# zovoilis-lab/Flye

Measured on AMD Instinct MI355X. Metric: Gbp reads overlapped/sec, higher is better.
Workload: dtype u64

## Files before the change

### flye_amd/csrc/fg_api.hip

```cpp
#include "fg_ctx.h"
#include <chrono>
#include <cmath>

#include <algorithm>
#include <new>

#include <mutex>
#include <atomic>

static std::mutex g_poolMutex;
static std::vector<BatchOwner*> g_pool;

BatchOwner* BatchOwner::acquire()
{
	std::lock_guard<std::mutex> lock(g_poolMutex);
	if (g_pool.empty()) return new BatchOwner;
	BatchOwner* b = g_pool.back();
	g_pool.pop_back();
	return b;
}

void BatchOwner::release(BatchOwner* b)
{
	if (!b) return;
// ... 562 lines not shown
		n > (1ULL << 40))
		return FG_ERR_ARG;
	return guarded(c, [&]()
	{
		HIP_CHECK(hipSetDevice(c->device));
		fgDebugScan(c, data, n, elem_bytes, inclusive != 0, in_place != 0);
	});
}

int fg_debug_radix_sort_pairs(fg_ctx* c, uint64_t* keys, uint64_t* vals, uint64_t n, int begin_bit, int end_bit,
							  int* passes_run)
{
	if (!c || (n && (!keys || !vals)) || begin_bit < 0 || end_bit > 64 || begin_bit > end_bit || n > (1ULL << 30) - 1 ||
		((uintptr_t)keys & 7u) || ((uintptr_t)vals & 7u))
		return FG_ERR_ARG;
	if (passes_run) *passes_run = 0;
	return guarded(c, [&]()
	{
		HIP_CHECK(hipSetDevice(c->device));
		fgDebugRadixSortPairs(c, keys, vals, n, begin_bit, end_bit, passes_run);
	});
}

int fg_debug_probe_skip_check(fg_ctx* c, uint64_t* clear_bits, uint64_t* violations)
{
	if (!c || !clear_bits || !violations) return FG_ERR_ARG;
	return guarded(c, [&]()
	{
		HIP_CHECK(hipSetDevice(c->device));
		if (!c->indexBuilt) throw FgError{FG_ERR_STATE, "no index"};
		u64 cb = 0, vi = 0;
		fgDebugProbeSkipCheck(c, &cb, &vi);
		*clear_bits = cb; *violations = vi;
	});
}

int fg_debug_edit_distances(fg_ctx* c, uint32_t n_pairs, int use_hpc, int32_t* out_dist, int32_t* out_len_a,
							int32_t* out_len_b)
{
	if (!c || (n_pairs && (!out_dist || !out_len_a || !out_len_b))) return FG_ERR_ARG;
	return guarded(c, [&]()
	{
		HIP_CHECK(hipSetDevice(c->device));
		fgDebugEditDistances(c, n_pairs, use_hpc, out_dist, out_len_a, out_len_b);
	});
}

namespace {
struct CigarOwner {
	std::vector<uint64_t> runOff;
	std::vector<uint8_t> ops;
	std::vector<int32_t> lens;
	std::vector<float> err;
};
}

int fg_align_cigar_ksw(fg_ctx* c, uint32_t n_pairs, const uint8_t* trg, const uint64_t* trg_off, const uint8_t* qry,
					   const uint64_t* qry_off, struct fg_cigar_batch* out)
{
	if (!c || !out || !trg_off || !qry_off || (trg_off[n_pairs] && !trg) || (qry_off[n_pairs] && !qry)) return FG_ERR_ARG;
	memset(out, 0, sizeof(*out));
	CigarOwner* own = nullptr;
	const int rc = guarded(c, [&]()
	{
		HIP_CHECK(hipSetDevice(c->device));
		std::vector<u64> runOff;
// ... 692 lines not shown
```

### flye_amd/csrc/fg_chain.hip

```cpp
#include "fg_wavesort.h"

#include <algorithm>

#define WG 256
#define I32_MIN ((i32)0x80000000)

struct ChainParams {
	int k, maxJump, minOverlap, maxOverhang;
	int checkOverhang, forceLocal;
	float minUnique;
	u32 firstId;
	u32 qFirstId;
	int onlyMaxExt;
	int keepAln;
	int ablate;
};

namespace {

struct CandAcc {
	typedef int4 T;
	int4* c;
	__device__ int4 load(int i) const { return c[i]; }
	__device__ void store(int i, const int4& x) { c[i] = x; }
	__device__ bool less(const int4& a, const int4& b) const { return a.w > b.w; }
};

__device__ __forceinline__ bool overlap_test(const ChainParams& P, u32 curId, u32 extId, i32 curLen,
											 i32 extLen, i32 cb, i32 ce, i32 eb, i32 ee)
{
	const i32 curRange = ce - cb, extRange = ee - eb;
	if (curRange < P.minOverlap || extRange < P.minOverlap) return false;
	const float lengthDiff = (float)abs(curRange - extRange);
	if (lengthDiff > 0.5f * (float)min(curRange, extRange)) return false;
	if (curId == extId)
	{
		const i32 inter = min(ce, ee) - max(cb, eb);
		if (inter > curRange / 2) return false;
	}
	if (curId == (extId ^ 1u))
	{
		const i32 inter = min(ce, extLen - eb) - max(cb, extLen - ee);
		if (inter > curRange / 2) return false;
	}
	if (!P.forceLocal && P.checkOverhang)
	{
		const i32 ovh = max(min(cb, eb), min(curLen - ce, extLen - ee));
		if (ovh > P.maxOverhang) return false;
// ... 431 lines not shown
			}
			else
			{
#pragma unroll
				for (int r = 0; r < R; ++r)
				{
					const u32 o = (u32)__shfl_xor((int)v[r], j);
					const bool asc = (((r * 64 + lane) & k) == 0);
					const bool lower = (lane & j) == 0;
					v[r] = (asc == lower) ? min(v[r], o) : max(v[r], o);
				}
			}
		}
	}
	bool tie = false;
	i32 nLive = 0;
#pragma unroll
	for (int r = 0; r < R; ++r)
	{
		u32 nx = (u32)__shfl_down((int)v[r], 1);
		const u32 first = r + 1 < R ? (u32)__builtin_amdgcn_readlane((int)v[r + 1 < R ? r + 1 : r], 0) : 0xFFFFFFFFu;
		if (lane == 63) nx = first;
		tie |= nx != 0xFFFFFFFFu && (nx >> 10) == (v[r] >> 10);
		nLive += __popcll(__builtin_amdgcn_ballot_w64(v[r] != 0xFFFFFFFFu));
	}
	if (__builtin_amdgcn_ballot_w64(tie)) return -1;
#pragma unroll
	for (int r = 0; r < R; ++r)
		if (v[r] != 0xFFFFFFFFu) oval[r * 64 + lane] = v[r] & 1023u;
	return nLive;
}


template <bool USE_LDS, int BT_CAP>
__device__ __forceinline__ void finish_group(const ChainParams& P, const i32 n, const u32 curId, const u32 extId, const i32 curLen,
											 const i32 extLen, const u32* cur, const u32* ext, i32* score, i32* back, u32* okey, u32* oval,
											 unsigned short* plLds, int* stack, int* small, i32* btLds, int4* cd, u32* primCountG)
{
	const int lane = threadIdx.x & 63;
	const int k = P.k;
	i32 nOrder = -1;
	if (USE_LDS && !(P.ablate & 64))
	{
		if (n <= 64) nOrder = fast_score_order<1>(n, score, back, oval);
		else if (n <= 128) nOrder = fast_score_order<2>(n, score, back, oval);
		else if (n <= 256) nOrder = fast_score_order<4>(n, score, back, oval);
	}
	const bool exact = nOrder < 0;
	if (exact)
	{
		for (i32 i = lane; i < n; i += 64) { okey[i] = (u32)(0x7fffffff - score[i]); oval[i] = (u32)i; }
		nOrder = n;
	}
	wsort::wave_mem_fence();
	if (exact && !(P.ablate & 2))
	{
		if (USE_LDS)
			wsort::wave_sort<u32, unsigned short>(okey, oval, n, plLds, plLds + n, stack, small);
		else if (BT_CAP > 0 && n <= BT_CAP)
		{
			unsigned short* pl = (unsigned short*)btLds;
			wsort::wave_sort<u32, unsigned short>(okey, oval, n, pl, pl + BT_CAP, stack, small);
		}
		else wsort::wave_sort<u32, u32>(okey, oval, n, oval + n, oval + 2 * n, stack, small);
	}

	if (P.ablate & 8) return;
	if (!USE_LDS && P.keepAln)
	{
		i32* bc = (i32*)(oval + n);
		for (i32 i = lane; i < n; i += 64) bc[i] = back[i];
		back = bc;
	}
// ... 269 lines not shown

u32 fetchU32(fg_ctx* c, const u32* dptr)
{
	u32 v;
	HIP_CHECK(hipMemcpyAsync(&v, dptr, 4, hipMemcpyDeviceToHost, c->stream));
	HIP_CHECK(hipStreamSynchronize(c->stream));
	return v;
}

}

u32 fgChainSmallMax()
{
	if (getenv("FG_CHAIN_FUSED") && atoi(getenv("FG_CHAIN_FUSED")) == 0) return 0u;
	return getenv("FG_FUSED_CAP") ? (u32)std::max(64, std::min(1024, atoi(getenv("FG_FUSED_CAP")))) : (u32)FIN_CAP_S;
}

void fgChainStage(fg_ctx* c, const fg_detector_params* p, uint8_t forceLocal, u64 nGroups, u64 nHits, int keyMode,
				  int curBits)
{
	hipStream_t s = c->stream;
	ChainParams cp;
	cp.k = c->k; cp.maxJump = p->max_jump; cp.minOverlap = p->min_overlap; cp.maxOverhang = p->max_overhang;
	cp.checkOverhang = p->max_overhang > 0; cp.forceLocal = forceLocal ? 1 : 0;
	{
		const float minKmerSruvivalRate = 0.01;
		cp.minUnique = minKmerSruvivalRate * p->min_overlap;
	}
	cp.firstId = c->firstId;
	cp.qFirstId = c->hasQ ? c->qFirstId : c->firstId;
	cp.onlyMaxExt = p->only_max_ext ? 1 : 0;
	cp.keepAln = p->keep_alignment ? 1 : 0;
	cp.ablate = getenv("FG_ABLATE") ? atoi(getenv("FG_ABLATE")) : 0;
	if (!nGroups) return;
	const i32* qLen = c->hasQ ? c->dQLen.p : c->dLen.p;
	u32 minSize = 0;
	while ((float)minSize < cp.minUnique) ++minSize;
	if (minSize == 0) minSize = 1;
	c->dListSmall.reserve(nGroups + 1); c->dListBig.reserve(nGroups + 1); c->dListDp.reserve(nGroups + 1);
	c->dGroupExtSorted.reserve(nGroups + 1);
	c->dListCnt.reserve(4);
	const u64 hitCap = std::max<u64>(nHits, c->hitCapHint);
	c->dCur.reserve(hitCap + 16); c->dExt.reserve(hitCap + 16);
	c->dScore.reserve(hitCap + 16); c->dBack.reserve(hitCap + 16);
	c->dTmp32.reserve(4 * hitCap + 16);
	c->dCand.reserve(hitCap + 1);
	const unsigned gridG = (unsigned)((nGroups + (u64)WG * LIST_ITEMS - 1) / ((u64)WG * LIST_ITEMS));
	const u32 fusedMax = fgChainSmallMax();
	const bool fused = fusedMax != 0;
	if (fused) c->dListFused.reserve(nGroups + 1);
	HIP_CHECK(hipMemsetAsync(c->dListCnt.p, 0, 16, s));
	{ ScopedK t(c->timer, "k_group_list");
	  hipLaunchKernelGGL(k_group_list, gridG, WG, 0, s, nGroups, nHits, c->dGroupStart.p, minSize, c->dGroupFirstCur.p,
						 c->dGroupLastCur.p, (i32)p->min_overlap, c->dListSmall.p, c->dListBig.p, (u32)PREP_CAP,
						 c->dListFused.p, fusedMax, c->dListCnt.p, c->dPrimFlag.p, c->dDpSize.p); }
	u32 nPrep[4];
	c->hScalar.reserve(8);
	HIP_CHECK(hipMemcpyAsync(c->hScalar.p, c->dListCnt.p, 16, hipMemcpyDeviceToHost, s));
	HIP_CHECK(hipStreamSynchronize(s));
	memcpy(nPrep, c->hScalar.p, 16);
	const u32 nFused = fused ? nPrep[2] : 0u;
	if (!nPrep[0] && !nPrep[1] && !nFused) return;
	if (fused)
	{
		const bool others = nPrep[0] || nPrep[1];
		const bool sideStreams = !(getenv("FG_CHAIN_STREAMS") && atoi(getenv("FG_CHAIN_STREAMS")) == 1);
// ... 199 lines not shown
```

### flye_amd/csrc/fg_ctx.h

```cpp
#pragma once

#include <hip/hip_runtime.h>
#include <cstdint>
#include <cstdio>
#include <cstdlib>
#include <new>
#include <cstring>
#include <string>
#include <vector>
#include <map>
#include <memory>
#include <condition_variable>
#include <functional>
#include <mutex>
#include <thread>
#include <atomic>
#include <algorithm>

#include "../../include/flye_gpu.h"

typedef uint64_t u64;
typedef uint32_t u32;
typedef int32_t i32;

// ... 281 lines not shown
	u64 hitCapHint = 0;
	const u32* curQuery = nullptr;
	DevBuf<u64> dQKmerOff;
	DevBuf<u64> dProbe;
	DevBuf<u64> dPartK0, dPartV0, dPartK1, dPartV1;
	DevBuf<char> dPartScratch;
	DevBuf<unsigned long long> dPartCount;
	DevBuf<u64> dHitOff;
	DevBuf<u64> dFiltOff;
	DevBuf<i32> dFiltPos;
	DevBuf<u64> dHitKey;
	DevBuf<u32> dHitVal;
	DevBuf<u32> dHitKey32;
	DevBuf<i32> dScore, dBack;
	DevBuf<int4> dCand;
	DevBuf<u64> dGroupStart;
	DevBuf<u32> dGroupQuery;
	DevBuf<u32> dGroupExt, dGroupFirstCur, dGroupLastCur;
	DevBuf<uint8_t> dGroupExtSorted;
	DevBuf<u32> dTmp32;
	DevBuf<fg_seed_hit> dSeedHits;
	DevBuf<u64> dRecvRun, dRecvIdx;
	DevBuf<u32> dRecvErr;
	DevBuf<u64> dCntA, dCntB, dGroupCnt, dGroupOff, dPrimCnt, dPrimOff, dDpGroups, dDpElems;
	DevBuf<u32> dPrimFlag, dDpSize, dListSmall, dListBig, dListDp, dListFused, dListCnt;
	DevBuf<u32> dCur, dExt;
	DevBuf<char> dPrimOut;
	DevBuf<u64> dPrimNode, dPrimBase, dMatchSize, dMatchOff, dMatches;
	DevBuf<u32> dMatchCnt;
	PinnedBuf<u64> hMatches, hMatchOff;
	PinnedBuf<u32> hMatchCnt;
	DevBuf<char> dSortTasks, dSortBig;
	DevBuf<unsigned long long> dSmallElems;
	DevBuf<u32> dSortCnt;
	DevBuf<u32> dTieFree;
	u32 tieFreeQ0 = 0, tieFreeN = 0;
	DevBuf<int> dEditScratch;
	DevBuf<u32> dEditList;
	DevBuf<char> dEditCnt;
	DevBuf<u64> dEditSlab;
	DevBuf<char> dEditPrims;
	DevBuf<u32> dEditQuery;
	DevBuf<i32> dEditOut;
	DevBuf<char> dRangeSides;
	DevBuf<i32> dRangeLen;
	DevBuf<u64> dRangeOff;
	DevBuf<uint8_t> dRangeTrg, dRangeQry;
	DevBuf<u32> dDecCnt;
	DevBuf<u64> dDecOff;
	DevBuf<uint8_t> dDecOps;
	DevBuf<i32> dDecLens;
	DevBuf<i32> dTrimPre;
	DevBuf<u64> dTrimRowCnt, dTrimRowOff, dTrimScan, dTrimKeys, dTrimIvl, dTrimSeg, dTrimAcc, dTrimAccOff;
	DevBuf<unsigned long long> dTrimPairCnt;
	DevBuf<u32> dTrimVals, dTrimAccCnt, dTrimKept;
	DevBuf<char> dTrimRaw, dTrimOut;
	DevBuf<u32> dRcNodes, dRcVals, dRcU32;
	DevBuf<char> dRcTab, dRcAln;
	DevBuf<u64> dRcOff, dRcKeys, dRcOut;
	DevBuf<i32> dRcOutScore;
	DevBuf<char> dCovRecs, dCovSort;
	DevBuf<u64> dCovIv, dCovKeys, dCovOff;
	DevBuf<i32> dCovI32, dCovVec;
	DevBuf<char> dPolBytes, dPolCand, dPolItems, dPolTasks, dPolRes;
	DevBuf<u64> dPolOff, dPolEdOff;
	DevBuf<long long> dPolScore, dPolCells, dPolEdits;
// ... 249 lines not shown
void fgKswAlign(fg_ctx* c, u32 nPairs, const uint8_t* trg, const u64* trgOff, const uint8_t* qry, const u64* qryOff,
				std::vector<u64>& runOff, std::vector<u32>& runs);
struct FgRangeSide { u32 rec; u32 flags; i32 start, len; };
void fgAlignRanges(fg_ctx* c, const std::vector<FgRangeSide>& sides, bool useHpc, std::vector<u64>& runOff,
				   std::vector<uint8_t>& ops, std::vector<i32>& lens, std::vector<u32>& errBases, std::vector<i32>& lenCur,
				   std::vector<i32>& lenExt);
struct FgDecodedRuns { u32 first, count; const u64* off; u64 nOut; };
void fgAlignRangesDevice(fg_ctx* c, const std::vector<FgRangeSide>& sides, bool useHpc, std::vector<u64>& runOff,
						 std::vector<u32>& errBases, std::vector<i32>& lenCur, std::vector<i32>& lenExt,
						 const std::function<void(const FgDecodedRuns&)>& sink);
void fgTrimRanges(fg_ctx* c, const std::vector<FgRangeSide>& sides, bool useHpc, float maxDivergence, i32 minOverlap,
				  std::vector<u64>& recOff, std::vector<fg_trim_rec>& recs);
void fgSortSegments(fg_ctx* c, const u64* dSegOff, u32 nSeg, u64* dKeys, u32* dVals, u64 n);
void fgEditRanges(fg_ctx* c, const std::vector<FgRangeSide>& sides, bool useHpc, i32* dist, i32* lenCur, i32* lenExt);
struct FgChainAln { i32 curBegin, curEnd, extBegin, extEnd, extLen, score; u32 ext; };
void fgChainAlignments(fg_ctx* c, const fg_chain_params& p, const std::vector<FgChainAln>& tab, const std::vector<u64>& qOff,
					   u64 recBase, const u32* nodeLeft, const u32* nodeRight, u32 nExt, std::vector<u64>& chainOff,
					   std::vector<u64>& alnOff, std::vector<u64>& aln, std::vector<i32>& score);
struct FgCovEdgeEl { i32 extBegin, extEnd; u32 edge, flags; };
void fgReadCoverage(fg_ctx* c, i32 window, i32 maxOverhang, i32 maxFlank, const fg_overlap_rec* recs, const std::vector<u64>& qOff,
					const std::vector<u64>& winOff, const std::vector<i32>& nClip, bool wantVectors, i32* full, i32* junction,
					long long* sum, i32* stat);
void fgEdgeCoverage(fg_ctx* c, i32 window, const std::vector<FgCovEdgeEl>& el, const std::vector<u64>& winOff, bool wantVectors,
					i32* cov, long long* sum, i32* stat);
void fgPolishBubbles(fg_ctx* c, const int64_t* score36, const uint8_t* cand, const uint64_t* candOff, const uint8_t* branches,
					 const uint64_t* branchOff, const uint64_t* bubbleBranchOff, u32 nBubbles, bool fixDinucleotides, bool wantSteps,
					 std::vector<std::string>& outCand, std::vector<uint32_t>& nSteps, std::vector<uint8_t>& status,
					 std::vector<std::vector<std::pair<std::string, int64_t>>>& steps);
void fgDebugSortPairs(fg_ctx* c, u64* keys, u32* vals, const u64* segOff, u32 nSeg);
void fgDebugSortPairs32(fg_ctx* c, u32* keys, u32* vals, const u64* segOff, u32 nSeg, int curBits, int recBits,
						const u32* tieFree, u64* radixSegments, u64* radixHits);
void fgDebugTieFree(fg_ctx* c, u32* out, u32 maxN, u32* firstQuery, u32* n);
void fgDebugProbeSkipCheck(fg_ctx* c, u64* clearBits, u64* violations);
void fgDebugEditDistances(fg_ctx* c, u32 nPairs, int useHpc, i32* outDist, i32* outLenA, i32* outLenB);
struct RecvHits {
	u32 nSrc;
	const u64* runStart;
	const u64* runLen;
	const u64* total;
	const fg_seed_hit* hits;
};
void fgOverlaps(fg_ctx* c, const fg_detector_params* p, const u32* queryIds, u32 nq, i32 maxOverlaps,
				uint8_t forceLocal, fg_overlap_batch* out, const RecvHits* recv = nullptr);
void fgIndexKeepTargets(fg_ctx* c, u32 world, u32 rank, u64* nKept);
#define FG_SPLIT_MAX_WORLD 128
void fgIndexPieceSplit(fg_ctx* c, u32 world, const u64** dCounts, const u64** dEntries, u64* destTotals);
void fgIndexScatterBegin(fg_ctx* c, u32 world, u32 rank, u64 nKeys, u64 nShardEntries, u64 nRep, u64** full);
void fgIndexScatterEnd(fg_ctx* c, float sampleRate);
void fgProbeHits(fg_ctx* c, const u32* queryIds, u32 nq, u64* hitCounts, const fg_seed_hit** dHits, u64* nHits);
void fgOverlapsFromHits(fg_ctx* c, const fg_detector_params* p, const u32* queryIds, u32 nq, i32 maxOverlaps,
						uint8_t forceLocal, u32 nSrc, const u64* hitCounts, const fg_seed_hit* dHits, fg_overlap_batch* out);
void fgFreqAccumulate(fg_ctx* c, u32* dst, const u32* src, u64 n);
void fgDebugFreqAccumulate(fg_ctx* c, u32* dst, const u32* src, u64 n);
int fgCheckOverlapArgs(const fg_ctx* c, const fg_detector_params* p, const u32* queryIds, u32 nq, i32 maxOverlaps);
void fgDebugScan(fg_ctx* c, void* data, u64 n, int elemBytes, bool inclusive, bool inPlace);
void fgDebugRadixSortPairs(fg_ctx* c, u64* keys, u64* vals, u64 n, int beginBit, int endBit, int* passesRun);
```

### flye_amd/csrc/fg_overlap.hip

```cpp
#include "fg_ctx.h"
#include "fg_wavesort.h"
#include "fg_devprim.h"
#include "fg_taskchain.h"
#include <atomic>

#include <algorithm>
#include <cmath>
#include <chrono>
#include <functional>
#include <thread>
#include <type_traits>

#define WG 256
#define FLAG_SELF (1ULL << 63)
#define FLAG_FLIP (1ULL << 62)
#define OFF_MASK ((1ULL << 38) - 1)

namespace {

__device__ __forceinline__ u32 block_exscan(u32 v, u32* sh , u32* total)
{
	const int lane = threadIdx.x & 63, w = threadIdx.x >> 6;
	u32 inc = v;
	for (int o = 1; o < 64; o <<= 1)
// ... 1164 lines not shown
		const u64 bit = kbase + (u64)p;
		if ((maybeBits[bit >> 5] >> (bit & 31)) & 1u) continue;
		++clear;
		u64 fw, rv;
		fg_kmer_pair(w, p, k, fw, rv);
		if (fg_probe<WIDE>(table, fw < rv ? fw : rv) != 0) ++bad;
	}
	for (int o = 32; o > 0; o >>= 1) { clear += __shfl_down(clear, o); bad += __shfl_down(bad, o); }
	if ((threadIdx.x & 63) == 0)
	{
		if (clear) atomicAdd(&out[0], (unsigned long long)clear);
		if (bad) atomicAdd(&out[1], (unsigned long long)bad);
	}
}

void fgDebugProbeSkipCheck(fg_ctx* c, u64* clearBits, u64* violations)
{
	*clearBits = *violations = 0;
	if (!c->dMaybeBits.p || !c->nReads) return;
	hipStream_t s = c->stream;
	DevBuf<unsigned long long> out;
	out.alloc(2);
	HIP_CHECK(hipMemsetAsync(out.p, 0, 16, s));
	if (c->tableWide)
		hipLaunchKernelGGL(k_probe_skip_check<true>, c->nReads, WG, 0, s, c->dWords.p, c->dWordOff.p, c->dLen.p, c->dKmerOff.p, c->k,
						   c->table, c->dMaybeBits.p, out.p);
	else
		hipLaunchKernelGGL(k_probe_skip_check<false>, c->nReads, WG, 0, s, c->dWords.p, c->dWordOff.p, c->dLen.p, c->dKmerOff.p, c->k,
						   c->table, c->dMaybeBits.p, out.p);
	unsigned long long h[2] = {0, 0};
	HIP_CHECK(hipMemcpyAsync(h, out.p, 16, hipMemcpyDeviceToHost, s));
	HIP_CHECK(hipStreamSynchronize(s));
	*clearBits = h[0]; *violations = h[1];
}

void fgSortSegments(fg_ctx* c, const u64* dSegOff, u32 nSeg, u64* dKeys, u32* dVals, u64 n)
{
	if (nSeg && n) sortSegments<u64>(c, dSegOff, nSeg, dKeys, dVals, n);
}

void fgDebugSortPairs(fg_ctx* c, u64* keys, u32* vals, const u64* segOff, u32 nSeg)
{
	hipStream_t s = c->stream;
	const u64 n = segOff[nSeg];
	DevBuf<u64> dK, dOff; DevBuf<u32> dV;
	dK.alloc(n + 1); dV.alloc(n + 1); dOff.alloc(nSeg + 1);
	HIP_CHECK(hipMemcpyAsync(dK.p, keys, n * 8, hipMemcpyHostToDevice, s));
	HIP_CHECK(hipMemcpyAsync(dV.p, vals, n * 4, hipMemcpyHostToDevice, s));
	HIP_CHECK(hipMemcpyAsync(dOff.p, segOff, (nSeg + 1) * 8ULL, hipMemcpyHostToDevice, s));
	if (nSeg) sortSegments<u64>(c, dOff.p, nSeg, dK.p, dV.p, n);
	HIP_CHECK(hipMemcpyAsync(keys, dK.p, n * 8, hipMemcpyDeviceToHost, s));
	HIP_CHECK(hipMemcpyAsync(vals, dV.p, n * 4, hipMemcpyDeviceToHost, s));
	HIP_CHECK(hipStreamSynchronize(s));
}

void fgDebugSortPairs32(fg_ctx* c, u32* keys, u32* vals, const u64* segOff, u32 nSeg, int curBits, int recBits,
						const u32* tieFree, u64* radixSegments, u64* radixHits)
{
	hipStream_t s = c->stream;
	const u64 n = segOff[nSeg];
	*radixSegments = *radixHits = 0;
	DevBuf<u32> dK, dV, dFlag; DevBuf<u64> dOff;
	dK.alloc(n + 1); dV.alloc(n + 1); dOff.alloc(nSeg + 1); dFlag.alloc(nSeg + 1);
	HIP_CHECK(hipMemcpyAsync(dK.p, keys, n * 4, hipMemcpyHostToDevice, s));
	HIP_CHECK(hipMemcpyAsync(dV.p, vals, n * 4, hipMemcpyHostToDevice, s));
	HIP_CHECK(hipMemcpyAsync(dOff.p, segOff, (nSeg + 1) * 8ULL, hipMemcpyHostToDevice, s));
// ... 338 lines not shown
}

static fg_ctx* laneTwo(fg_ctx* c)
{
	if (!c->lane2)
	{
		std::unique_ptr<fg_ctx> l(new fg_ctx);
		l->device = c->device;
		if (hipStreamCreateWithFlags(&l->stream, hipStreamNonBlocking) != hipSuccess ||
			hipStreamCreateWithFlags(&l->stream2, hipStreamNonBlocking) != hipSuccess ||
			hipStreamCreateWithFlags(&l->stream3, hipStreamNonBlocking) != hipSuccess ||
			hipEventCreateWithFlags(&l->evJoin3, hipEventDisableTiming) != hipSuccess ||
			hipEventCreateWithFlags(&l->evOff, hipEventDisableTiming) != hipSuccess ||
			hipEventCreateWithFlags(&l->evFork, hipEventDisableTiming) != hipSuccess ||
			hipEventCreateWithFlags(&l->evJoin, hipEventDisableTiming) != hipSuccess)
			throw FgError{FG_ERR_HIP, "streams of the second lane"};
		for (auto& e : l->evPiece)
			if (hipEventCreateWithFlags(&e, hipEventDisableTiming) != hipSuccess) throw FgError{FG_ERR_HIP, "events of the second lane"};
		l->timer.stream = l->stream;
		c->lane2 = std::move(l);
	}
	fg_ctx* l = c->lane2.get();
	l->k = c->k; l->nReads = c->nReads; l->firstId = c->firstId; l->maxLen = c->maxLen;
	l->totalKmers = c->totalKmers; l->totalBases = c->totalBases;
	l->hasQ = c->hasQ; l->nQReads = c->nQReads; l->qFirstId = c->qFirstId; l->qMaxLen = c->qMaxLen;
	l->indexBuilt = c->indexBuilt; l->sampleRate = c->sampleRate; l->nKeys = c->nKeys; l->nEntries = c->nEntries; l->nRep = c->nRep;
	l->tableSlots = c->tableSlots; l->tableWide = c->tableWide; l->table = c->table;
	l->timer.enabled = c->timer.enabled;
	l->dWords.alias(c->dWords); l->dWordOff.alias(c->dWordOff); l->dLen.alias(c->dLen); l->dKmerOff.alias(c->dKmerOff);
	l->dQWords.alias(c->dQWords); l->dQWordOff.alias(c->dQWordOff); l->dQLen.alias(c->dQLen);
	l->dKeyOff.alias(c->dKeyOff); l->dEntries.alias(c->dEntries); l->dTable.alias(c->dTable); l->dIndexedBits.alias(c->dIndexedBits); l->dMaybeBits.alias(c->dMaybeBits);
	l->dQuery.alias(c->dQuery); l->dQKmerOff.alias(c->dQKmerOff); l->dProbe.alias(c->dProbe);
	l->dCntA.alias(c->dCntA); l->dCntB.alias(c->dCntB);
	return l;
}

struct SubResult {
	u32 qa = 0, qb = 0;
	int lane = 0;
	u64 lanePrimBase = 0;
	ChunkResult cr{};
	std::vector<u64> primOff;
	std::vector<u64> mData, mOff;
};

void fgOverlaps(fg_ctx* c, const fg_detector_params* p, const u32* queryIds, u32 nq, i32 maxOverlaps,
				uint8_t forceLocal, fg_overlap_batch* out, const RecvHits* recv)
{
	hipStream_t s = c->stream;
	const int k = c->k;
	c->timer.reset();
	c->hitCapHint = 0;
	const auto tHost0 = std::chrono::steady_clock::now();
	struct EvPair {
		KernelTimer& t; hipEvent_t a, b;
		explicit EvPair(KernelTimer& t_) : t(t_), a(t_.get()), b(nullptr) { try { b = t_.get(); } catch (...) { t_.pool.push_back(a); throw; } }
		~EvPair() { t.pool.push_back(a); t.pool.push_back(b); }
	} evp(c->timer);
	const hipEvent_t evA = evp.a, evB = evp.b;
	HIP_CHECK(hipEventRecord(evA, s));

	BatchOwner* own = BatchOwner::acquire();
	out->owner_ = own;
	out->n_queries = nq;
	own->queryOff.assign(nq + 1, 0);
	own->statOff.assign(nq + 1, 0);

	std::vector<u32> hq(nq);
	std::vector<u64> hQKmerOff(nq + 1, 0);
	u64 queryBp = 0;
	const int STAT_WND = 10000;
	u64 statCap = 0;
	for (u32 i = 0; i < nq; ++i)
	{
		hq[i] = queryIds[i] - (c->hasQ ? c->qFirstId : c->firstId);
		const i32 L = (c->hasQ ? c->hQLen : c->hLen)[hq[i] >> 1];
		hQKmerOff[i + 1] = hQKmerOff[i] + (u64)std::max(0, L - k);
		queryBp += L;
		statCap += (u64)(L / STAT_WND + 1);
	}
	out->query_bp = queryBp;
	out->query_kmers = hQKmerOff[nq];
	if (nq == 0)
	{
		out->query_off = own->queryOff.data(); out->div_stats_off = own->statOff.data();
		if (p->keep_alignment) { own->matchOff.assign(1, 0); out->match_off = own->matchOff.data(); }
		if (p->partition_bad_mappings) { own->needsTrim.assign(1, 0); out->needs_trim = own->needsTrim.data(); }
		return;
	}
#ifdef FG_SORT_ABLATE
	if (getenv("FG_ABLATE"))
	{
		const int ab = atoi(getenv("FG_ABLATE"));
// ... 415 lines not shown
```

### flye_amd/gpu.py

```python
from __future__ import annotations

import ctypes as C
import os

import time

import numpy as np

_HERE = os.path.dirname(os.path.abspath(__file__))
LIB_PATH = os.environ.get("FLYE_GPU_LIB") or os.path.join(_HERE, "lib", "libflyegpu.so")

REC_DTYPE = np.dtype([("cur_id", "<u4"), ("ext_id", "<u4"), ("cur_begin", "<i4"),
                      ("cur_end", "<i4"), ("cur_len", "<i4"), ("ext_begin", "<i4"),
                      ("ext_end", "<i4"), ("ext_len", "<i4"), ("score", "<i4"),
                      ("seq_divergence", "<f4"), ("chain_length", "<i4"),
                      ("filtered_positions", "<i4"), ("edit_distance", "<i4"),
                      ("hpc_len_cur", "<i4"), ("hpc_len_ext", "<i4")])

ABI_SYMBOLS = ["fg_abi_version", "fg_create", "fg_destroy", "fg_strerror", "fg_last_error",
               "fg_container_info", "fg_set_reads", "fg_set_queries", "fg_build_index_solid", "fg_build_index_minimizers",
               "fg_index_begin_solid", "fg_index_begin_minimizers", "fg_index_build_range", "fg_index_finish",
               "fg_index_kmer_hist", "fg_index_count_slice", "fg_index_batch_freq", "fg_index_batch_select",
               "fg_index_selection_done", "fg_index_gather_begin", "fg_index_gather_end", "fg_memory_stats",
               "fg_import_index", "fg_index_device_arrays", "fg_clear_index", "fg_export_index", "fg_overlaps", "fg_release_batch",
               "fg_kernel_times", "fg_debug_sort_pairs", "fg_debug_edit_distances", "fg_align_cigar_ksw", "fg_release_cigars",
               "fg_align_ranges", "fg_trim_ranges", "fg_release_trims", "fg_edit_ranges", "fg_chain_divergence",
               "fg_chain_alignments", "fg_release_chains",
               "fg_read_coverage", "fg_release_coverage", "fg_coverage_windows", "fg_coverage_verdict",
               "fg_edge_coverage", "fg_release_edge_coverage",
               "fg_subs_matrix_load", "fg_polish_bubbles", "fg_release_polish", "fg_make_bubbles", "fg_release_bubbles",
               "fg_uniform_alignments", "fg_release_uniform", "fg_contig_consensus", "fg_release_consensus",
               "fg_index_keep_targets", "fg_index_shard", "fg_probe_hits", "fg_overlaps_from_hits",
               "fg_index_piece_split", "fg_index_scatter_begin", "fg_index_scatter_end", "fg_debug_probe_skip_check",
               "fg_group_create", "fg_group_destroy", "fg_group_size", "fg_group_member", "fg_group_last_error",
               "fg_group_set_reads", "fg_group_set_queries", "fg_group_build_index_solid",
               "fg_group_build_index_minimizers", "fg_group_clear_index", "fg_group_overlaps", "fg_group_stats",
               "fg_group_build_info", "fg_debug_freq_accumulate", "fg_debug_group_bin_cuts", "fg_debug_scan",
               "fg_debug_radix_sort_pairs", "fg_debug_tie_free"]

RANGE_PAIR_DTYPE = np.dtype([("cur_id", "<u4"), ("ext_id", "<u4"), ("cur_begin", "<i4"), ("cur_end", "<i4"),
                             ("ext_begin", "<i4"), ("ext_end", "<i4")])

TRIM_REC_DTYPE = np.dtype([("cur_begin", "<i4"), ("cur_end", "<i4"), ("ext_begin", "<i4"), ("ext_end", "<i4"),
                           ("run_start", "<i4"), ("run_end", "<i4"), ("range_err", "<i4"), ("range_len", "<i4"),
                           ("seq_divergence", "<f4")])

SEED_HIT_DTYPE = np.dtype([("cur_pos", "<i4"), ("ext_pos", "<i4"), ("ext_id", "<u4")])


class FlyeGpuError(RuntimeError):
    def __init__(self, code, msg):
        super().__init__(f"libflyegpu error {code}: {msg}")
        self.code = code


class IndexStats(C.Structure):
    _fields_ = [("total_kmers", C.c_uint64), ("selected_kmers", C.c_uint64),
                ("index_entries", C.c_uint64), ("repetitive_kmers", C.c_uint64),
                ("repetitive_frequency", C.c_uint64), ("mean_frequency", C.c_float),
                ("sample_rate", C.c_float), ("build_seconds", C.c_double)]

    def as_dict(self):
        return {k: getattr(self, k) for k, _ in self._fields_}


class DetectorParams(C.Structure):
    _fields_ = [("max_jump", C.c_int32), ("min_overlap", C.c_int32),
                ("max_overhang", C.c_int32), ("keep_alignment", C.c_uint8),
                ("only_max_ext", C.c_uint8), ("nucl_alignment", C.c_uint8),
                ("partition_bad_mappings", C.c_uint8), ("use_hpc", C.c_uint8),
                ("pad_", C.c_uint8 * 3), ("max_divergence", C.c_float)]
# ... 167 lines not shown
        L.fg_index_finish.argtypes = [C.c_void_p, C.c_void_p, C.POINTER(IndexStats)]
        L.fg_index_kmer_hist.argtypes = [C.c_void_p, C.c_void_p]
        L.fg_index_count_slice.argtypes = [C.c_void_p, C.c_int32, C.c_float, C.c_int32, C.c_float, C.c_float, C.c_uint32,
                                           C.c_uint32, C.POINTER(C.c_uint64), C.POINTER(C.c_uint32)]
        L.fg_index_batch_freq.argtypes = [C.c_void_p, C.c_uint32, C.POINTER(C.c_void_p), C.POINTER(C.c_uint64)]
        L.fg_index_batch_select.argtypes = [C.c_void_p, C.c_uint32]
        L.fg_index_selection_done.argtypes = [C.c_void_p, C.c_void_p]
        L.fg_index_gather_begin.argtypes = [C.c_void_p, C.c_uint64, C.c_uint64, C.c_uint64, C.c_void_p, C.c_void_p, C.c_void_p]
        L.fg_index_gather_end.argtypes = [C.c_void_p, C.c_float]
        L.fg_memory_stats.argtypes = [C.POINTER(C.c_uint64), C.POINTER(C.c_uint64), C.c_int]
        L.fg_import_index.argtypes = [C.c_void_p, C.c_uint64, C.c_void_p, C.c_void_p, C.c_uint64, C.c_void_p, C.c_uint64,
                                      C.c_void_p, C.c_float, C.c_int]
        L.fg_index_device_arrays.argtypes = [C.c_void_p] + [C.c_void_p] * 7
        L.fg_clear_index.argtypes = [C.c_void_p]
        L.fg_export_index.argtypes = [C.c_void_p] + [C.c_void_p] * 7
        L.fg_overlaps.argtypes = [C.c_void_p, C.POINTER(DetectorParams), C.c_void_p, C.c_uint32,
                                  C.c_int32, C.c_uint8, C.POINTER(OverlapBatch)]
        L.fg_release_batch.argtypes = [C.POINTER(OverlapBatch)]
        L.fg_index_keep_targets.argtypes = [C.c_void_p, C.c_uint32, C.c_uint32, C.POINTER(C.c_uint64)]
        L.fg_index_shard.argtypes = [C.c_void_p, C.POINTER(C.c_uint32), C.POINTER(C.c_uint32)]
        L.fg_index_piece_split.argtypes = [C.c_void_p, C.c_uint32, C.POINTER(C.c_void_p), C.POINTER(C.c_void_p), C.c_void_p]
        L.fg_index_scatter_begin.argtypes = [C.c_void_p, C.c_uint32, C.c_uint32, C.c_uint64, C.c_uint64, C.c_uint64, C.c_void_p]
        L.fg_index_scatter_end.argtypes = [C.c_void_p, C.c_float]
        L.fg_probe_hits.argtypes = [C.c_void_p, C.c_void_p, C.c_uint32, C.c_void_p, C.POINTER(C.c_void_p),
                                    C.POINTER(C.c_uint64)]
        L.fg_overlaps_from_hits.argtypes = [C.c_void_p, C.POINTER(DetectorParams), C.c_void_p, C.c_uint32, C.c_int32,
                                            C.c_uint8, C.c_uint32, C.c_void_p, C.c_void_p, C.POINTER(OverlapBatch)]
        L.fg_kernel_times.argtypes = [C.c_void_p, C.POINTER(KernelTime), C.c_int]
        L.fg_debug_sort_pairs.argtypes = [C.c_void_p, C.c_void_p, C.c_void_p, C.c_void_p, C.c_uint32]
        L.fg_debug_sort_pairs32.argtypes = [C.c_void_p, C.c_void_p, C.c_void_p, C.c_void_p, C.c_uint32, C.c_int, C.c_int,
                                            C.c_void_p, C.POINTER(C.c_uint64), C.POINTER(C.c_uint64)]
        L.fg_debug_tie_free.argtypes = [C.c_void_p, C.c_void_p, C.c_uint32, C.POINTER(C.c_uint32), C.POINTER(C.c_uint32)]
        L.fg_debug_probe_skip_check.argtypes =[C.c_void_p, C.POINTER(C.c_uint64), C.POINTER(C.c_uint64)]
        L.fg_debug_edit_distances.argtypes = [C.c_void_p, C.c_uint32, C.c_int, C.c_void_p, C.c_void_p, C.c_void_p]
        L.fg_align_cigar_ksw.argtypes = [C.c_void_p, C.c_uint32, C.c_void_p, C.c_void_p, C.c_void_p, C.c_void_p,
                                         C.POINTER(CigarBatch)]
        L.fg_release_cigars.argtypes = [C.POINTER(CigarBatch)]
        L.fg_align_ranges.argtypes = [C.c_void_p, C.c_void_p, C.c_uint32, C.c_uint8, C.POINTER(CigarBatch), C.c_void_p,
                                      C.c_void_p]
        L.fg_trim_ranges.argtypes = [C.c_void_p, C.c_void_p, C.c_uint32, C.c_uint8, C.c_float, C.c_int32, C.POINTER(TrimBatch)]
        L.fg_release_trims.argtypes = [C.POINTER(TrimBatch)]
        L.fg_release_trims.restype = None
        L.fg_edit_ranges.argtypes = [C.c_void_p, C.c_void_p, C.c_uint32, C.c_uint8, C.c_void_p, C.c_void_p, C.c_void_p,
                                     C.c_void_p]
        L.fg_chain_divergence.argtypes = [C.c_void_p, C.c_void_p, C.c_void_p, C.c_uint32, C.c_void_p]
        L.fg_chain_alignments.argtypes = [C.c_void_p, C.POINTER(ChainParams), C.c_void_p, C.c_void_p, C.c_uint32, C.c_uint32,
                                          C.c_uint32, C.c_void_p, C.c_void_p, C.POINTER(ChainBatch)]
        L.fg_release_chains.argtypes = [C.POINTER(ChainBatch)]
        L.fg_release_chains.restype = None
        L.fg_read_coverage.argtypes = [C.c_void_p, C.POINTER(CoverageParams), C.c_void_p, C.c_void_p, C.c_uint32, C.c_void_p,
                                       C.POINTER(CoverageBatch)]
        L.fg_release_coverage.argtypes = [C.POINTER(CoverageBatch)]
        L.fg_release_coverage.restype = None
        L.fg_coverage_windows.argtypes = [C.c_int32, C.c_int32, C.c_int32, C.POINTER(C.c_int32), C.POINTER(C.c_int32),
                                          C.POINTER(C.c_uint8)]
        L.fg_coverage_verdict.argtypes = [C.POINTER(CoverageParams), C.c_uint32, C.c_void_p, C.c_void_p, C.c_void_p, C.c_void_p,
                                          C.c_void_p, C.c_void_p]
        L.fg_edge_coverage.argtypes = [C.c_void_p, C.c_int32, C.c_void_p, C.c_uint64, C.c_void_p, C.c_void_p, C.c_uint64,
                                       C.c_uint32, C.c_uint32, C.c_void_p, C.c_uint32, C.c_void_p, C.c_uint8,
                                       C.POINTER(EdgeCoverageBatch)]
        L.fg_release_edge_coverage.argtypes = [C.POINTER(EdgeCoverageBatch)]
        L.fg_release_edge_coverage.restype = None
        L.fg_subs_matrix_load.argtypes = [C.c_char_p, C.POINTER(SubsMatrixStruct)]
        L.fg_polish_bubbles.argtypes = [C.c_void_p, C.POINTER(SubsMatrixStruct), C.c_void_p, C.c_void_p, C.c_void_p, C.c_void_p,
                                        C.c_void_p, C.c_uint32, C.c_uint8, C.c_uint8, C.POINTER(PolishBatch)]
        L.fg_release_polish.argtypes = [C.POINTER(PolishBatch)]
# ... 344 lines not shown
        self._check(self.L.fg_debug_tie_free(self.h, out.ctypes.data, int(max_n), C.byref(q0), C.byref(n)))
        if n.value > max_n:
            raise ValueError(f"{n.value} flags, room for {max_n}")
        return int(q0.value), out[:n.value].copy()

    def debug_freq_accumulate(self, dst, src):
        assert dst.dtype == np.uint32 and src.dtype == np.uint32 and len(dst) == len(src)
        assert dst.flags.c_contiguous and src.flags.c_contiguous
        self._check(self.L.fg_debug_freq_accumulate(self.h, dst.ctypes.data, src.ctypes.data, len(dst)))
        return dst

    def debug_scan(self, data, inclusive=False, in_place=True):
        assert data.dtype in (np.uint32, np.uint64)
        out = np.ascontiguousarray(data).copy()
        self._check(self.L.fg_debug_scan(self.h, out.ctypes.data if len(out) else None, len(out), out.dtype.itemsize,
                                         int(bool(inclusive)), int(bool(in_place))))
        return out

    def debug_radix_sort_pairs(self, keys, vals, begin_bit, end_bit):
        k = np.ascontiguousarray(keys, np.uint64).copy()
        v = np.ascontiguousarray(vals, np.uint64).copy()
        assert len(k) == len(v)
        passes = C.c_int(-1)
        self._check(self.L.fg_debug_radix_sort_pairs(self.h, k.ctypes.data if len(k) else None,
                                                     v.ctypes.data if len(v) else None, len(k), begin_bit, end_bit,
                                                     C.byref(passes)))
        return k, v, int(passes.value)

    def debug_probe_skip_check(self):
        clear, bad = C.c_uint64(0), C.c_uint64(0)
        self._check(self.L.fg_debug_probe_skip_check(self.h, C.byref(clear), C.byref(bad)))
        return int(clear.value), int(bad.value)

    def debug_edit_distances(self, n_pairs, use_hpc=False):
        d = np.empty(n_pairs, np.int32)
        la = np.empty(n_pairs, np.int32)
        lb = np.empty(n_pairs, np.int32)
        self._check(self.L.fg_debug_edit_distances(self.h, n_pairs, int(bool(use_hpc)), d.ctypes.data,
                                                   la.ctypes.data, lb.ctypes.data))
        return d, la, lb

    def align_cigar_ksw(self, pairs, arrays=False):
        n = len(pairs)
        trg = np.concatenate([np.asarray(a, np.uint8) for a, _ in pairs]) if n else np.empty(0, np.uint8)
        qry = np.concatenate([np.asarray(b, np.uint8) for _, b in pairs]) if n else np.empty(0, np.uint8)
        toff = np.zeros(n + 1, np.uint64)
        qoff = np.zeros(n + 1, np.uint64)
        toff[1:] = np.cumsum([len(a) for a, _ in pairs])
        qoff[1:] = np.cumsum([len(b) for _, b in pairs])
        trg = np.ascontiguousarray(trg if len(trg) else np.zeros(1, np.uint8))
        qry = np.ascontiguousarray(qry if len(qry) else np.zeros(1, np.uint8))
        b = CigarBatch()
        t0 = time.perf_counter()
        self._check(self.L.fg_align_cigar_ksw(self.h, n, trg.ctypes.data, toff.ctypes.data, qry.ctypes.data,
                                              qoff.ctypes.data, C.byref(b)))
        self.last_align_seconds = time.perf_counter() - t0
        out = self._cigar_result(b, n, arrays)
        self.L.fg_release_cigars(C.byref(b))
        return out

    @staticmethod
    def _cigar_result(b, n, arrays):
        run_off = np.ctypeslib.as_array(b.run_off, (n + 1,)).copy() if n else np.zeros(1, np.uint64)
        total = int(run_off[n])
        ops = np.ctypeslib.as_array(b.ops, (total,)).copy() if total else np.empty(0, np.uint8)
        lens = np.ctypeslib.as_array(b.lens, (total,)).copy() if total else np.empty(0, np.int32)
# ... 1137 lines not shown
```

### include/flye_gpu.h

```cpp
#ifndef FLYE_GPU_H
#define FLYE_GPU_H

#include <stdint.h>

#ifdef __cplusplus
extern "C" {
#endif

#define FG_ABI_VERSION 4

enum {
	FG_OK = 0,
	FG_ERR_NO_DEVICE = -1,
	FG_ERR_HIP = -2,
	FG_ERR_ARG = -3,
	FG_ERR_STATE = -4,
	FG_ERR_KMER_TOO_FREQUENT = -5,
	FG_ERR_KMER_SIZE = -6,
	FG_ERR_UNSUPPORTED = -7,
	FG_ERR_NOMEM = -8
};

typedef struct fg_ctx fg_ctx;

// ... 155 lines not shown
int fg_group_overlaps(fg_group* g, const struct fg_detector_params* p, const uint32_t* query_ids,
                      uint32_t n_queries, int32_t max_overlaps, uint8_t force_local,
                      struct fg_overlap_batch* out);
struct fg_group_stats { uint64_t hits_moved_bytes, hits_total, peer_copies; double exchange_seconds; };
int fg_group_stats(const fg_group* g, struct fg_group_stats* out);
struct fg_group_build_info {
	uint32_t selection_batches, stage_pieces_max;
	uint64_t stage_pieces, freq_bytes, scatter_bytes;
};
int fg_group_build_info(const fg_group* g, struct fg_group_build_info* out);

struct fg_kernel_time { const char* name; double seconds; uint64_t launches; };
int fg_kernel_times(fg_ctx* ctx, struct fg_kernel_time* out, int max_entries);

int fg_debug_sort_pairs(fg_ctx* ctx, uint64_t* keys, uint32_t* vals,
                        const uint64_t* seg_off, uint32_t n_seg);

int fg_debug_sort_pairs32(fg_ctx* ctx, uint32_t* keys, uint32_t* vals, const uint64_t* seg_off, uint32_t n_seg,
                          int cur_bits, int rec_bits, const uint32_t* tie_free,
                          uint64_t* radix_segments, uint64_t* radix_hits);

int fg_debug_tie_free(fg_ctx* ctx, uint32_t* out, uint32_t max_n, uint32_t* first_query, uint32_t* n);

int fg_debug_group_bin_cuts(const uint64_t* hist, uint32_t world, uint32_t* cuts);

int fg_debug_freq_accumulate(fg_ctx* ctx, uint32_t* dst, const uint32_t* src, uint64_t n);

int fg_debug_scan(fg_ctx* ctx, void* data, uint64_t n, int elem_bytes, int inclusive, int in_place);

int fg_debug_radix_sort_pairs(fg_ctx* ctx, uint64_t* keys, uint64_t* vals, uint64_t n, int begin_bit, int end_bit,
                              int* passes_run);

int fg_debug_probe_skip_check(fg_ctx* ctx, uint64_t* clear_bits, uint64_t* violations);

int fg_debug_edit_distances(fg_ctx* ctx, uint32_t n_pairs, int use_hpc, int32_t* out_dist,
                            int32_t* out_len_a, int32_t* out_len_b);

struct fg_cigar_batch {
	uint32_t  n_pairs;
	uint64_t* run_off;
	uint8_t*  ops;
	int32_t*  lens;
	float*    err_rate;
	void*     owner_;
};
int fg_align_cigar_ksw(fg_ctx* ctx, uint32_t n_pairs, const uint8_t* trg, const uint64_t* trg_off,
                       const uint8_t* qry, const uint64_t* qry_off, struct fg_cigar_batch* out);
void fg_release_cigars(struct fg_cigar_batch* b);

struct fg_range_pair { uint32_t cur_id, ext_id; int32_t cur_begin, cur_end, ext_begin, ext_end; };
int fg_align_ranges(fg_ctx* ctx, const struct fg_range_pair* pairs, uint32_t n_pairs, uint8_t use_hpc,
                    struct fg_cigar_batch* out, int32_t* len_cur, int32_t* len_ext);

struct fg_trim_rec {
	int32_t cur_begin, cur_end, ext_begin, ext_end;
	int32_t run_start, run_end;
	int32_t range_err, range_len;
	float   seq_divergence;
};
struct fg_trim_batch { uint32_t n_pairs; uint64_t* rec_off; struct fg_trim_rec* recs; void* owner_; };
int fg_trim_ranges(fg_ctx* ctx, const struct fg_range_pair* pairs, uint32_t n_pairs, uint8_t use_hpc,
                   float max_divergence, int32_t min_overlap, struct fg_trim_batch* out);
void fg_release_trims(struct fg_trim_batch* b);

int fg_edit_ranges(fg_ctx* ctx, const struct fg_range_pair* pairs, uint32_t n_pairs, uint8_t use_hpc,
                   int32_t* dist, int32_t* len_cur, int32_t* len_ext, float* divergence);
// ... 173 lines not shown
```

Before: 4.483.

## Add lazy fast path extracting the single best chain without sorting

When only the maximal extension is needed, each group first finds the unique top-scoring chain end with a wave reduction. It then walks back pointers, using pointer jumping in LDS or a windowed walk through global memory, and emits that one primary if it passes the overlap test. This skips the full score sort and backtrack in finish_group. Ties, roots that are not index 0, and failed overlap tests fall back to the exact path. The change also adds per-wave atomic counters and a debug API for fast-path statistics, which cost one atomic per wave on every group.

```diff
diff --git a/flye_amd/csrc/fg_api.hip b/flye_amd/csrc/fg_api.hip
--- a/flye_amd/csrc/fg_api.hip
+++ b/flye_amd/csrc/fg_api.hip
@@ -618,6 +618,18 @@
 		u64 cb = 0, vi = 0;
 		fgDebugProbeSkipCheck(c, &cb, &vi);
 		*clear_bits = cb; *violations = vi;
+	});
+}
+
+int fg_debug_chain_lazy(fg_ctx* c, uint64_t out[6])
+{
+	if (!c || !out) return FG_ERR_ARG;
+	return guarded(c, [&]()
+	{
+		HIP_CHECK(hipSetDevice(c->device));
+		u64 h[6];
+		fgDebugChainLazy(c, h);
+		for (int i = 0; i < 6; ++i) out[i] = h[i];
 	});
 }
 
diff --git a/flye_amd/csrc/fg_chain.hip b/flye_amd/csrc/fg_chain.hip
--- a/flye_amd/csrc/fg_chain.hip
+++ b/flye_amd/csrc/fg_chain.hip
@@ -14,6 +14,8 @@
 	int onlyMaxExt;
 	int keepAln;
 	int ablate;
+	int lazy;
+	unsigned long long* lazyCnt;
 };
 
 namespace {
@@ -511,6 +513,101 @@
 }
 
 
+enum { LZ_ENTERED = 0, LZ_FAST, LZ_NOLIVE, LZ_TIE, LZ_ROOT, LZ_TEST, LZ_ROW = 8 };
+__device__ __forceinline__ void lazy_count(const ChainParams& P, int what)
+{
+	if ((threadIdx.x & 63) == 0)
+		atomicAdd(&P.lazyCnt[(size_t)(blockIdx.x & (FG_LAZY_STRIPES - 1)) * LZ_ROW + what], 1ULL);
+}
+
+template <bool USE_LDS, int BT_CAP>
+__device__ __forceinline__ bool lazy_primary(const ChainParams& P, const i32 n, const u32 curId, const u32 extId, const i32 curLen,
+											 const i32 extLen, const u32* cur, const u32* ext, const i32* score, const i32* back,
+											 i32* stage, u32* ja, u32* jb, int4* cd, u32* primCountG)
+{
+	const int lane = threadIdx.x & 63;
+	const bool staged = !USE_LDS && BT_CAP > 0 && n <= BT_CAP;
+	i32 bs = I32_MIN, bi = 0;
+	bool tie = false, toZero = false;
+#pragma unroll 4
+	for (i32 i = lane; i < n; i += 64)
+	{
+		i32 b, s;
+		if (USE_LDS)
+		{
+			b = back[i]; s = score[i];
+			ja[i] = b == -1 ? (u32)i << 16 : ((u32)b << 16) | 1u;
+		}
+		else
+		{
+			b = __hip_atomic_load(&back[i], __ATOMIC_RELAXED, __HIP_MEMORY_SCOPE_AGENT);
+			s = __hip_atomic_load(&score[i], __ATOMIC_RELAXED, __HIP_MEMORY_SCOPE_AGENT);
+			if (staged) stage[i] = b;
+		}
+		toZero |= b == 0;
+		if (b != -1)
+		{
+			tie = s == bs ? true : (s > bs ? false : tie);
+			bi = s > bs ? i : bi;
+			bs = max(bs, s);
+		}
+	}
+	const i32 top = __builtin_amdgcn_readlane(wave_incl_max(bs), 63);
+	if (top == I32_MIN) { lazy_count(P, LZ_NOLIVE); return true; }
+	const u64 topM = __builtin_amdgcn_ballot_w64(bs == top);
+	if ((topM & (topM - 1)) || __builtin_amdgcn_ballot_w64(tie && bs == top)) { lazy_count(P, LZ_TIE); return false; }
+	const i32 last = __builtin_amdgcn_readlane(bi, __builtin_amdgcn_readfirstlane(__ffsll((long long)topM) - 1));
+	const bool anyToZero = __builtin_amdgcn_ballot_w64(toZero) != 0;
+	i32 first = last, chainLength = 0;
+	if (USE_LDS)
+	{
+		u32 *src = ja, *dst = jb;
+		wsort::wave_mem_fence();
+		while (true)
+		{
+			const u32 w = fg_uni(src[last]), a = w >> 16;
+			if ((fg_uni(src[a]) >> 16) == a) { first = (i32)a; chainLength = (i32)(w & 0xffffu) + 1; break; }
+			for (i32 i = lane; i <= last; i += 64)
+			{
+				const u32 w1 = src[i], w2 = src[w1 >> 16];
+				dst[i] = (w2 & 0xffff0000u) | ((w1 + w2) & 0xffffu);
+			}
+			wsort::wave_mem_fence();
+			u32* t = src; src = dst; dst = t;
+		}
+	}
+	else
+	{
+		if (staged) wsort::wave_mem_fence();
+		i32 wbase = -0x40000000, win = -1, pos = last;
+		while (true)
+		{
+			if (pos < wbase || pos >= wbase + 64)
+			{
+				wbase = max(0, pos - 63);
+				if (staged) win = wbase + lane < n ? stage[wbase + lane] : -1;
+				else win = wbase + lane < n ? __hip_atomic_load(&back[wbase + lane], __ATOMIC_RELAXED, __HIP_MEMORY_SCOPE_AGENT) : -1;
+			}
+			const i32 np = __builtin_amdgcn_readlane(win, __builtin_amdgcn_readfirstlane(pos - wbase));
+			first = pos;
+			++chainLength;
+			if (np == -1) break;
+			pos = np;
+		}
+	}
+	if (first != 0 && anyToZero) { lazy_count(P, LZ_ROOT); return false; }
+	const i32 cb = (i32)cur[first], eb = (i32)ext[first];
+	const i32 ce = (i32)cur[last] + P.k - 1, ee = (i32)ext[last] + P.k - 1;
+	if (!overlap_test(P, curId, extId, curLen, extLen, cb, ce, eb, ee)) { lazy_count(P, LZ_TEST); return false; }
+	if (lane == 0)
+	{
+		cd[0] = make_int4(first, last, chainLength, top - score[first] + P.k - 1);
+		*primCountG = 1;
+	}
+	lazy_count(P, LZ_FAST);
+	return true;
+}
+
 template <bool USE_LDS, int BT_CAP>
 __device__ __forceinline__ void finish_group(const ChainParams& P, const i32 n, const u32 curId, const u32 extId, const i32 curLen,
 											 const i32 extLen, const u32* cur, const u32* ext, i32* score, i32* back, u32* okey, u32* oval,
@@ -518,6 +615,9 @@
 {
 	const int lane = threadIdx.x & 63;
 	const int k = P.k;
+	lazy_count(P, LZ_ENTERED);
+	if (P.lazy && lazy_primary<USE_LDS, BT_CAP>(P, n, curId, extId, curLen, extLen, cur, ext, score, back, btLds, okey, oval, cd, primCountG))
+		return;
 	i32 nOrder = -1;
 	if (USE_LDS && !(P.ablate & 64))
 	{
@@ -853,6 +953,8 @@
 	cp.onlyMaxExt = p->only_max_ext ? 1 : 0;
 	cp.keepAln = p->keep_alignment ? 1 : 0;
 	cp.ablate = getenv("FG_ABLATE") ? atoi(getenv("FG_ABLATE")) : 0;
+	cp.lazy = cp.onlyMaxExt && !(getenv("FG_CHAIN_LAZY") && atoi(getenv("FG_CHAIN_LAZY")) == 0);
+	cp.lazyCnt = c->dLazyCnt.p;
 	if (!nGroups) return;
 	const i32* qLen = c->hasQ ? c->dQLen.p : c->dLen.p;
 	u32 minSize = 0;
diff --git a/flye_amd/csrc/fg_ctx.h b/flye_amd/csrc/fg_ctx.h
--- a/flye_amd/csrc/fg_ctx.h
+++ b/flye_amd/csrc/fg_ctx.h
@@ -337,6 +337,7 @@
 	PinnedBuf<u32> hMatchCnt;
 	DevBuf<char> dSortTasks, dSortBig;
 	DevBuf<unsigned long long> dSmallElems;
+	DevBuf<unsigned long long> dLazyCnt;
 	DevBuf<u32> dSortCnt;
 	DevBuf<u32> dTieFree;
 	u32 tieFreeQ0 = 0, tieFreeN = 0;
@@ -652,6 +653,8 @@
 						const u32* tieFree, u64* radixSegments, u64* radixHits);
 void fgDebugTieFree(fg_ctx* c, u32* out, u32 maxN, u32* firstQuery, u32* n);
 void fgDebugProbeSkipCheck(fg_ctx* c, u64* clearBits, u64* violations);
+#define FG_LAZY_STRIPES 64
+void fgDebugChainLazy(fg_ctx* c, u64 out[6]);
 void fgDebugEditDistances(fg_ctx* c, u32 nPairs, int useHpc, i32* outDist, i32* outLenA, i32* outLenB);
 struct RecvHits {
 	u32 nSrc;
diff --git a/flye_amd/csrc/fg_overlap.hip b/flye_amd/csrc/fg_overlap.hip
--- a/flye_amd/csrc/fg_overlap.hip
+++ b/flye_amd/csrc/fg_overlap.hip
@@ -1220,6 +1220,17 @@
 	HIP_CHECK(hipMemcpyAsync(h, out.p, 16, hipMemcpyDeviceToHost, s));
 	HIP_CHECK(hipStreamSynchronize(s));
 	*clearBits = h[0]; *violations = h[1];
+}
+
+void fgDebugChainLazy(fg_ctx* c, u64 out[6])
+{
+	for (int i = 0; i < 6; ++i) out[i] = 0;
+	if (!c->dLazyCnt.p) return;
+	std::vector<unsigned long long> h((size_t)FG_LAZY_STRIPES * 8);
+	HIP_CHECK(hipMemcpyAsync(h.data(), c->dLazyCnt.p, h.size() * sizeof(unsigned long long), hipMemcpyDeviceToHost, c->stream));
+	HIP_CHECK(hipStreamSynchronize(c->stream));
+	for (int r = 0; r < FG_LAZY_STRIPES; ++r)
+		for (int i = 0; i < 6; ++i) out[i] += h[(size_t)r * 8 + i];
 }
 
 void fgSortSegments(fg_ctx* c, const u64* dSegOff, u32 nSeg, u64* dKeys, u32* dVals, u64 n)
@@ -1624,6 +1635,7 @@
 	l->dKeyOff.alias(c->dKeyOff); l->dEntries.alias(c->dEntries); l->dTable.alias(c->dTable); l->dIndexedBits.alias(c->dIndexedBits); l->dMaybeBits.alias(c->dMaybeBits);
 	l->dQuery.alias(c->dQuery); l->dQKmerOff.alias(c->dQKmerOff); l->dProbe.alias(c->dProbe);
 	l->dCntA.alias(c->dCntA); l->dCntB.alias(c->dCntB);
+	l->dLazyCnt.alias(c->dLazyCnt);
 	return l;
 }
 
@@ -1651,6 +1663,8 @@
 	} evp(c->timer);
 	const hipEvent_t evA = evp.a, evB = evp.b;
 	HIP_CHECK(hipEventRecord(evA, s));
+	c->dLazyCnt.reserve(FG_LAZY_STRIPES * 8);
+	HIP_CHECK(hipMemsetAsync(c->dLazyCnt.p, 0, FG_LAZY_STRIPES * 8 * sizeof(unsigned long long), s));
 
 	BatchOwner* own = BatchOwner::acquire();
 	out->owner_ = own;
diff --git a/flye_amd/gpu.py b/flye_amd/gpu.py
--- a/flye_amd/gpu.py
+++ b/flye_amd/gpu.py
@@ -36,7 +36,7 @@
                "fg_group_set_reads", "fg_group_set_queries", "fg_group_build_index_solid",
                "fg_group_build_index_minimizers", "fg_group_clear_index", "fg_group_overlaps", "fg_group_stats",
                "fg_group_build_info", "fg_debug_freq_accumulate", "fg_debug_group_bin_cuts", "fg_debug_scan",
-               "fg_debug_radix_sort_pairs", "fg_debug_tie_free"]
+               "fg_debug_radix_sort_pairs", "fg_debug_tie_free", "fg_debug_chain_lazy"]
 
 RANGE_PAIR_DTYPE = np.dtype([("cur_id", "<u4"), ("ext_id", "<u4"), ("cur_begin", "<i4"), ("cur_end", "<i4"),
                              ("ext_begin", "<i4"), ("ext_end", "<i4")])
@@ -270,6 +270,7 @@
                                             C.c_void_p, C.POINTER(C.c_uint64), C.POINTER(C.c_uint64)]
         L.fg_debug_tie_free.argtypes = [C.c_void_p, C.c_void_p, C.c_uint32, C.POINTER(C.c_uint32), C.POINTER(C.c_uint32)]
         L.fg_debug_probe_skip_check.argtypes =[C.c_void_p, C.POINTER(C.c_uint64), C.POINTER(C.c_uint64)]
+        L.fg_debug_chain_lazy.argtypes = [C.c_void_p, C.POINTER(C.c_uint64)]
         L.fg_debug_edit_distances.argtypes = [C.c_void_p, C.c_uint32, C.c_int, C.c_void_p, C.c_void_p, C.c_void_p]
         L.fg_align_cigar_ksw.argtypes = [C.c_void_p, C.c_uint32, C.c_void_p, C.c_void_p, C.c_void_p, C.c_void_p,
                                          C.POINTER(CigarBatch)]
@@ -680,6 +681,11 @@
         self._check(self.L.fg_debug_probe_skip_check(self.h, C.byref(clear), C.byref(bad)))
         return int(clear.value), int(bad.value)
 
+    def debug_chain_lazy(self):
+        out = (C.c_uint64 * 6)()
+        self._check(self.L.fg_debug_chain_lazy(self.h, out))
+        return dict(zip(("entered", "fast", "no_live", "tied_top", "root", "overlap_test"), (int(x) for x in out)))
+
     def debug_edit_distances(self, n_pairs, use_hpc=False):
         d = np.empty(n_pairs, np.int32)
         la = np.empty(n_pairs, np.int32)
diff --git a/include/flye_gpu.h b/include/flye_gpu.h
--- a/include/flye_gpu.h
+++ b/include/flye_gpu.h
@@ -211,6 +211,8 @@
                               int* passes_run);
 
 int fg_debug_probe_skip_check(fg_ctx* ctx, uint64_t* clear_bits, uint64_t* violations);
+
+int fg_debug_chain_lazy(fg_ctx* ctx, uint64_t out[6]);
 
 int fg_debug_edit_distances(fg_ctx* ctx, uint32_t n_pairs, int use_hpc, int32_t* out_dist,
                             int32_t* out_len_a, int32_t* out_len_b);
```

Measured after the change: 4.788 (median of 6 runs). 1.07x the previous value.
